# norlab-ulaval/norlab_icp_mapper

Hardware: AMD Instinct MI355X
Metric: ICP iterations/sec, 100k-pt scan vs 1M-pt map (higher is better)
Workload: dtype f32; 1 GPU; single synthetic 100000-pt scan vs 1000000-pt map, point-to-point ICP, KDTreeMatcher knn 1 maxDist 2.0 epsilon 0, TrimmedDist 0.85, fixed 20 iterations per registration; chain=p2p, scene=box+pillars sigma=0.01 seeds 42/43/44 (SURVEY.md 8d), parallelism=scan-sharded x1, map replicated

## Files before the change

include/icpmi.h:

```cpp
#ifndef ICPMI_H
#define ICPMI_H

#include <stdint.h>

#ifdef __cplusplus
extern "C" {
#endif

#define ICPMI_VERSION 4

typedef struct icpmi_ctx* icpmi_handle;

typedef enum {
    ICPMI_OK = 0,
    ICPMI_ERR_INVALID_ARG = 1,
    ICPMI_ERR_HIP = 2,
    ICPMI_ERR_NO_POINT_TO_MINIMIZE = 3,
    ICPMI_ERR_NO_OUTLIER_TO_FILTER = 4,
    ICPMI_ERR_BOUND = 5,
    ICPMI_ERR_NAN = 6,
    ICPMI_ERR_MISSING_NORMALS = 7,
    ICPMI_ERR_UNSUPPORTED = 8
} icpmi_status;

// ... 39 lines not shown
    int32_t minimizer;
    int32_t force_4dof;
    int32_t force_2d;
    int32_t is_2d;
    int32_t max_iterations;
    int32_t use_differential;
    float   min_diff_rot;
    float   min_diff_trans;
    int32_t smooth_length;
    int32_t use_bound;
    float   max_rot_norm;
    float   max_trans_norm;
    float   grid_cell;
    int32_t use_graph;
    int32_t profile;
    int32_t fuse_solve;
    int32_t knn_wg_from;
    int32_t sel_window_off;
    int32_t epsilon_approx;
    int32_t covariance;
    float   sensor_std_dev;
    union {
        int32_t var_dist;
        int32_t reserved[2];
    };
} icpmi_config;

typedef struct {
    int32_t iterations;
    int32_t stop_reason;
    int64_t pairs;
// ... 190 lines not shown
```

norlab_icp_mapper_amd/_capi.py:

```python
import ctypes as C
import os

_HERE = os.path.dirname(os.path.abspath(__file__))
LIB_PATH = os.path.join(_HERE, "libicpmi.so")

ICPMI_OK = 0
ERR_INVALID_ARG, ERR_HIP, ERR_NO_POINT_TO_MINIMIZE, ERR_NO_OUTLIER_TO_FILTER = 1, 2, 3, 4
ERR_BOUND, ERR_NAN, ERR_MISSING_NORMALS, ERR_UNSUPPORTED = 5, 6, 7, 8
MIN_IDENTITY, MIN_POINT_TO_POINT, MIN_POINT_TO_PLANE = 0, 1, 2
OUT_MAXDIST, OUT_MINDIST, OUT_MEDIANDIST, OUT_TRIMMEDDIST, OUT_SURFACENORMAL = 1, 2, 3, 4, 5
OUT_GENERICDESCRIPTOR, OUT_ROBUST, OUT_VARTRIMMEDDIST = 6, 7, 8
GEN_SOURCE_READING, GEN_SOFT, GEN_LARGER = 1, 2, 4
ROBUST_FCT = {"cauchy": 0, "welsch": 1, "sc": 2, "gm": 3, "tukey": 4, "huber": 5, "L1": 6, "student": 7}
ROBUST_SCALE = {"none": 0, "mad": 1, "berg": 2, "std": 3}
ROBUST_DIST = {"point2point": 0, "point2plane": 1}
STOP_NONE, STOP_COUNTER, STOP_DIFFERENTIAL = 0, 1, 2


class Outlier(C.Structure):
    _fields_ = [("type", C.c_int32), ("param", C.c_float), ("iparam", C.c_int32), ("param2", C.c_float), ("param3", C.c_float)]


class _ConfigTail(C.Union):
    _fields_ = [("var_dist", C.c_int32), ("reserved", C.c_int32 * 2)]
# ... 11 lines not shown
        ("minimizer", C.c_int32),
        ("force_4dof", C.c_int32),
        ("force_2d", C.c_int32),
        ("is_2d", C.c_int32),
        ("max_iterations", C.c_int32),
        ("use_differential", C.c_int32),
        ("min_diff_rot", C.c_float),
        ("min_diff_trans", C.c_float),
        ("smooth_length", C.c_int32),
        ("use_bound", C.c_int32),
        ("max_rot_norm", C.c_float),
        ("max_trans_norm", C.c_float),
        ("grid_cell", C.c_float),
        ("use_graph", C.c_int32),
        ("profile", C.c_int32),
        ("fuse_solve", C.c_int32),
        ("knn_wg_from", C.c_int32),
        ("sel_window_off", C.c_int32),
        ("epsilon_approx", C.c_int32),
        ("covariance", C.c_int32),
        ("sensor_std_dev", C.c_float),
        ("tail", _ConfigTail),
    ]


class Stats(C.Structure):
    _fields_ = [
        ("iterations", C.c_int32),
        ("stop_reason", C.c_int32),
        ("pairs", C.c_int64),
        ("point_used_ratio", C.c_float),
# ... 134 lines not shown
```

norlab_icp_mapper_amd/csrc/api.hip:

```cpp
#include "common.h"
#include <cstring>
#include <new>
#include <dlfcn.h>
#include <mutex>
#include <cstdio>

static std::string g_create_error;

namespace {
struct Roctx {
    int (*push)(const char*) = nullptr;
    int (*pop)() = nullptr;
    Roctx()
    {
        const char* e = getenv("ICPMI_ROCTX");
        if (!e || !atoi(e)) return;
        for (const char* name : {"librocprofiler-sdk-roctx.so.1", "librocprofiler-sdk-roctx.so", "/opt/rocm/lib/librocprofiler-sdk-roctx.so.1",
                                 "libroctx64.so.4", "libroctx64.so", "/opt/rocm/lib/libroctx64.so.4"}) {
            void* lib = dlopen(name, RTLD_NOW | RTLD_GLOBAL);
            if (!lib) continue;
            push = (int (*)(const char*))dlsym(lib, "roctxRangePushA");
            pop = (int (*)())dlsym(lib, "roctxRangePop");
            if (push && pop) return;
            push = nullptr; pop = nullptr;
// ... 41 lines not shown
    cfg->n_outlier = 0;
    cfg->minimizer = ICPMI_MIN_POINT_TO_PLANE;
    cfg->max_iterations = 40;
    cfg->use_differential = 0;
    cfg->min_diff_rot = 0.001f;
    cfg->min_diff_trans = 0.001f;
    cfg->smooth_length = 3;
    cfg->use_bound = 0;
    cfg->max_rot_norm = 1.f;
    cfg->max_trans_norm = 1.f;
    cfg->grid_cell = 0.f;
    cfg->use_graph = 1;
    cfg->profile = 0;
    cfg->covariance = 0;
    cfg->sensor_std_dev = 0.01f;
}

static icpmi_status validate_config(const icpmi_config* cfg, std::string& err)
{
    if (cfg->knn < 1 || cfg->knn > ICPMI_MAX_K) { err = "InvalidParameter: knn must be in [1, 32]"; return ICPMI_ERR_INVALID_ARG; }
    if (cfg->var_dist != 0 && cfg->var_dist != 1) { err = "InvalidParameter: var_dist must be 0 or 1"; return ICPMI_ERR_INVALID_ARG; }
    if (!cfg->var_dist && !(cfg->max_dist > 0.f)) { err = "InvalidParameter: maxDist must be > 0"; return ICPMI_ERR_INVALID_ARG; }
    if (cfg->epsilon < 0.f) { err = "InvalidParameter: epsilon must be >= 0"; return ICPMI_ERR_INVALID_ARG; }
    if (cfg->n_outlier < 0 || cfg->n_outlier > ICPMI_MAX_OUTLIER) { err = "InvalidParameter: at most 8 outlier filters"; return ICPMI_ERR_INVALID_ARG; }
    for (int f = 0; f < cfg->n_outlier; ++f) {
        const int t = cfg->outlier[f].type;
        const float p = cfg->outlier[f].param;
        if (t < ICPMI_OUT_MAXDIST || t > ICPMI_OUT_VARTRIMMEDDIST) { err = "InvalidParameter: unknown outlier filter type"; return ICPMI_ERR_INVALID_ARG; }
        if (t == ICPMI_OUT_VARTRIMMEDDIST) {
            const float lo = cfg->outlier[f].param, hi = cfg->outlier[f].param2, lam = cfg->outlier[f].param3;
// ... 177 lines not shown

icpmi_status icpmi_debug_counters(icpmi_handle h, uint64_t out[24])
{
    if (!h || !out) return ICPMI_ERR_INVALID_ARG;
    for (int i = 0; i < 24; ++i) out[i] = h->h_state->dbg[i];
#ifndef ICPMI_NN_TIMING
    out[14] = (uint64_t)h->merge_fast_epochs;
    out[15] = (uint64_t)h->merge_slow_epochs;
    out[16] = (uint64_t)h->oct_respeculated;
    out[17] = (uint64_t)h->raw_view_count;
    out[18] = (uint64_t)(uint32_t)h->ins_count | ((uint64_t)(uint32_t)(h->temp_raw ? h->temp_raw->ins_count : 0) << 32);
    out[19] = (uint64_t)(uint32_t)h->full_count | ((uint64_t)(uint32_t)(h->temp_raw ? h->temp_raw->full_count : 0) << 32);
    out[20] = (uint64_t)h->normals_incremental;
    out[21] = (uint64_t)h->normals_full;
    out[22] = (uint64_t)h->normals_last_searched;
#endif
    return ICPMI_OK;
}

icpmi_status icpmi_debug_last_matches(icpmi_handle h, int64_t n, int32_t k, int32_t* ids, float* d2, float T_used[16])
{
    CHECK_H(h);
    if (n < 1 || k < 1 || !ids || !d2 || !T_used) { h->last_error = "debug_last_matches: bad arguments"; return ICPMI_ERR_INVALID_ARG; }
    if (h->last_match_n == 0) {
        h->last_error = "debug_last_matches: no single registration's matches on this handle (none ran, it failed, or a batch / another call came after it)";
        return ICPMI_ERR_UNSUPPORTED;
    }
    if (n != h->last_match_n || k != h->last_match_k) { h->last_error = "debug_last_matches: n / k differ from the last registration's"; return ICPMI_ERR_INVALID_ARG; }
    const size_t cnt = (size_t)n * k;
    DevBuf<int> d_ids;
// ... 934 lines not shown
```

norlab_icp_mapper_amd/csrc/common.h:

```cpp
#pragma once

#include <hip/hip_runtime.h>
#include <stdint.h>
#include <math.h>
#include <cstring>
#include <string>
#include <vector>
#include <unordered_map>
#include <mutex>
#include <map>
#include <cstdlib>
#include <shared_mutex>

#include "../../include/icpmi.h"

#define ICPMI_NV 32
#define ICPMI_MAX_OUTLIER 8
#define ICPMI_MAX_SMOOTH 16
#define ICPMI_SEL_BINS 2048
#ifndef ICPMI_S2_COPIES
#define ICPMI_S2_COPIES 8
#endif
#define ICPMI_S2_C0 4096
#define ICPMI_S2_F0 (ICPMI_S2_C0 + ICPMI_S2_COPIES * 256)
// ... 354 lines not shown
    bool own_stream = false;
    std::string last_error;
    std::recursive_mutex mu;

    int64_t m = 0;
    float mean[3] = {0, 0, 0};
    GridParams grid{};
    int64_t n_occupied = 0;
    DevArr<float4> d_map_sorted;
    DevArr<float4> d_normals_sorted;
    DevArr<float4> d_map_pn;
    DevArr<unsigned> d_cell_start;
    bool has_normals = false;
    GridLevels levels{};
    DevArr<uint4> d_lvl_tab;
    DevArr<float4> d_lvl_pts[ICPMI_MAXLEV];
    DevArr<unsigned> d_lvl_cs[ICPMI_MAXLEV];
    DevArr<unsigned> d_lvl_pos0[ICPMI_MAXLEV];
    DevArr<unsigned> d_inv;
    DevArr<unsigned> d_lvl_key[ICPMI_MAXLEV];
    DevArr<float4> d_alt_pts[ICPMI_MAXLEV];
    DevArr<unsigned> d_alt_cs[ICPMI_MAXLEV];
    DevArr<unsigned> d_alt_pos0[ICPMI_MAXLEV];
    DevArr<unsigned> d_alt_key[ICPMI_MAXLEV];
    DevArr<float4> d_raw0;
    DevArr<float4> d_alt_raw0;
    DevArr<unsigned> d_ins_dstart0;
    DevArr<float4> d_alt_nsorted;
    DevArr<float4> d_alt_pn;
    DevArr<unsigned> d_ins_key;
    DevArr<unsigned> d_ins_rank;
    bool ins_ready = false;
    bool ins_normals_changed = false;
    double sum_raw[3] = {0, 0, 0};
    float lo_raw[3] = {0, 0, 0}, hi_raw[3] = {0, 0, 0};
    float cell0 = 0.f;
    uint64_t raw_epoch = 0;
    uint64_t temp_raw_epoch = 0; int64_t temp_raw_m = 0;
    uint64_t raw_view_version = 0;
// ... 529 lines not shown
```

norlab_icp_mapper_amd/csrc/map_build.hip:

```cpp
#include "common.h"
#include <cstring>

namespace {

constexpr int RB = 256;

__global__ __launch_bounds__(RB) void stats_kernel(const float4* __restrict__ pts, int64_t m, double* __restrict__ part)
{
    double sx = 0, sy = 0, sz = 0;
    float lo[3] = {INFINITY, INFINITY, INFINITY}, hi[3] = {-INFINITY, -INFINITY, -INFINITY};
    for (int64_t i = (int64_t)blockIdx.x * RB + threadIdx.x; i < m; i += (int64_t)gridDim.x * RB) {
        const float4 p = pts[i];
        sx += p.x; sy += p.y; sz += p.z;
        lo[0] = fminf(lo[0], p.x); lo[1] = fminf(lo[1], p.y); lo[2] = fminf(lo[2], p.z);
        hi[0] = fmaxf(hi[0], p.x); hi[1] = fmaxf(hi[1], p.y); hi[2] = fmaxf(hi[2], p.z);
    }
    __shared__ double sh[RB * 3];
    __shared__ float shlo[RB * 3], shhi[RB * 3];
    const int t = threadIdx.x;
    sh[t] = sx; sh[RB + t] = sy; sh[2 * RB + t] = sz;
    for (int r = 0; r < 3; ++r) { shlo[r * RB + t] = lo[r]; shhi[r * RB + t] = hi[r]; }
    __syncthreads();
    for (int s = RB / 2; s > 0; s >>= 1) {
        if (t < s) {
// ... 731 lines not shown


static GridParams make_grid(const float lo[3], const float hi[3], float cell, float maxabs)
{
    GridParams g;
    g.ox = lo[0]; g.oy = lo[1]; g.oz = lo[2];
    g.cell = cell; g.inv_cell = 1.0f / cell;
    g.slack = cell * 1e-3f + maxabs * 2e-6f;
    g.nx = (int)floorf((hi[0] - lo[0]) * g.inv_cell) + 1;
    g.ny = (int)floorf((hi[1] - lo[1]) * g.inv_cell) + 1;
    g.nz = (int)floorf((hi[2] - lo[2]) * g.inv_cell) + 1;
    g.ncells = g.nx * g.ny * g.nz;
    return g;
}

icpmi_status upload_level_table(icpmi_ctx* c)
{
    GridLevels& L = c->levels;
    uint32_t tab[ICPMI_MAXLEV * 16] = {0};
    auto fbits = [](float f) { uint32_t u; memcpy(&u, &f, 4); return u; };
    for (int l = 0; l < L.nlev; ++l) {
        uint32_t* t = tab + 16 * l;
        const GridParams& gl = L.g[l];
        t[0] = fbits(gl.ox); t[1] = fbits(gl.oy); t[2] = fbits(gl.oz); t[3] = fbits(gl.cell);
        t[4] = fbits(gl.inv_cell); t[5] = fbits(gl.slack); t[6] = (uint32_t)gl.nx; t[7] = (uint32_t)gl.ny;
        t[8] = (uint32_t)gl.nz; t[9] = (uint32_t)gl.ncells;
        const uint64_t pp = (uint64_t)(uintptr_t)L.pts[l], pc = (uint64_t)(uintptr_t)L.cs[l], p0 = (uint64_t)(uintptr_t)L.pos0[l];
        t[10] = (uint32_t)pp; t[11] = (uint32_t)(pp >> 32);
        t[12] = (uint32_t)pc; t[13] = (uint32_t)(pc >> 32); t[14] = (uint32_t)p0; t[15] = (uint32_t)(p0 >> 32);
    }
    if (!c->d_lvl_tab) HIP_TRY(c, c->d_lvl_tab.alloc(ICPMI_MAXLEV * 4));
    return upload_small(c, c->d_lvl_tab, tab, sizeof tab);
}

static icpmi_status map_insert(icpmi_ctx* c, const float4* d_pts, int64_t m0, int64_t m1, const float* d_normals3, bool normals_changed, bool* done)
{
    *done = false;
    static int on = -1, min_m = -1;
    if (on < 0) { on = 1; const char* e = getenv("ICPMI_INSERT_MIN"); min_m = e ? atoi(e) : 0; }
    const int64_t n = m1 - m0;
    GridLevels& L = c->levels;
    if (!on || !c->ins_ready || m0 != c->m || m0 <= 0 || n <= 0 || n > m0 / 2 || m1 < min_m || (d_normals3 != nullptr) != c->has_normals || c->cfg.grid_cell > 0.f) return ICPMI_OK;
    if (c->keep_raw && (d_pts != c->d_raw || (d_normals3 && d_normals3 != c->d_raw_n3))) return ICPMI_OK;
    const int rblocks = (int)std::min<int64_t>((n + RB - 1) / RB, 256);
    if (c->d_red.ensure(c, (size_t)rblocks * 9) != ICPMI_OK) return ICPMI_ERR_HIP;
    hipLaunchKernelGGL(stats_kernel, dim3(rblocks), dim3(RB), 0, c->stream, d_pts + m0, n, c->d_red);
    HIP_TRY(c, hipGetLastError());
// ... 1 lines not shown
    if (read_back(c, part.data(), c->d_red, part.size() * sizeof(double)) != ICPMI_OK) return ICPMI_ERR_HIP;
    double sum[3] = {c->sum_raw[0], c->sum_raw[1], c->sum_raw[2]};
    for (int b = 0; b < rblocks; ++b)
        for (int r = 0; r < 3; ++r) {
            sum[r] += part[(size_t)b * 9 + r];
            const float lo = (float)part[(size_t)b * 9 + 3 + r], hi = (float)part[(size_t)b * 9 + 6 + r];
            const float over = 2.0f * c->levels.g[0].cell;
            if (!(lo >= c->lo_raw[r] - over) || !(hi <= c->hi_raw[r] + over)) return ICPMI_OK;
        }
    float mean[3], clo[3], chi[3], maxabs = 0.f;
    for (int r = 0; r < 3; ++r) {
        mean[r] = c->no_centre ? 0.f : (float)(sum[r] / (double)m1);
        clo[r] = c->lo_raw[r] - mean[r]; chi[r] = c->hi_raw[r] - mean[r];
        maxabs = fmaxf(maxabs, fmaxf(fabsf(clo[r]), fabsf(chi[r])));
    }
    GridParams gnew[ICPMI_MAXLEV];
    for (int l = 0; l < L.nlev; ++l) {
        gnew[l] = make_grid(clo, chi, L.g[l].cell, maxabs);
        if (gnew[l].nx != L.g[l].nx || gnew[l].ny != L.g[l].ny || gnew[l].nz != L.g[l].nz) return ICPMI_OK;
    }
    const bool with_n = d_normals3 != nullptr;
    const bool with_pn = with_n && c->d_map_pn != nullptr && !c->single_level && c->keep_raw;
    if (c->d_ins_key.ensure(c, (size_t)n + 1) != ICPMI_OK || c->d_ins_rank.ensure(c, (size_t)n + 1) != ICPMI_OK) return ICPMI_ERR_HIP;
    const bool twin = !c->no_centre;
    if (twin && !c->d_raw0) return ICPMI_OK;
    if (c->d_inv.ensure(c, (size_t)n + 1) != ICPMI_OK) return ICPMI_ERR_HIP;
    if (c->d_fill.ensure(c, (size_t)L.g[0].ncells + 2) != ICPMI_OK) return ICPMI_ERR_HIP;
    c->fill_clean = false;
    if (c->d_ins_dstart0.ensure(c, (size_t)L.g[0].ncells + 2) != ICPMI_OK) return ICPMI_ERR_HIP;
    if (twin && c->d_alt_raw0.ensure(c, (size_t)m1 + 16) != ICPMI_OK) return ICPMI_ERR_HIP;
    for (int l = 0; l < L.nlev; ++l) {
        if (c->d_alt_pts[l].ensure(c, (size_t)m1 + 16) != ICPMI_OK) return ICPMI_ERR_HIP;
        if (c->d_alt_key[l].ensure(c, (size_t)m1 + 1) != ICPMI_OK) return ICPMI_ERR_HIP;
        if (c->d_alt_cs[l].ensure(c, (size_t)L.g[l].ncells + 2) != ICPMI_OK) return ICPMI_ERR_HIP;
        if (l > 0 && c->d_alt_pos0[l].ensure(c, (size_t)m1 + 1) != ICPMI_OK) return ICPMI_ERR_HIP;
    }
    if (with_n && c->d_alt_nsorted.ensure(c, (size_t)m1 + 1) != ICPMI_OK) return ICPMI_ERR_HIP;
    if (with_pn && c->d_alt_pn.ensure(c, 2 * (size_t)m1 + 2) != ICPMI_OK) return ICPMI_ERR_HIP;
    const int gb0 = (int)((m0 + 255) / 256), gbn = (int)((n + 255) / 256);
    for (int l = 0; l < L.nlev; ++l) {
        const GridParams& g = gnew[l];
        float4* pts_old = l == 0 ? c->d_map_sorted : c->d_lvl_pts[l];
        unsigned* cs_old = l == 0 ? c->d_cell_start : c->d_lvl_cs[l];
        unsigned* key_old = c->d_lvl_key[l];
        unsigned* dstart = l == 0 ? c->d_ins_dstart0 : c->d_fill;
        HIP_TRY(c, hipMemsetAsync(dstart, 0, ((size_t)g.ncells + 2) * sizeof(unsigned), c->stream));
        hipLaunchKernelGGL(ins_key_kernel, dim3(gbn), dim3(256), 0, c->stream, d_pts, m0, n, mean[0], mean[1], mean[2], g, c->d_ins_key, c->d_ins_rank, dstart);
        if (device_exclusive_scan(c, dstart, g.ncells, (unsigned)n) != ICPMI_OK) return ICPMI_ERR_HIP;
        if (l == 0)
            hipLaunchKernelGGL(ins_move0_kernel, dim3(gb0), dim3(256), 0, c->stream, (const float4*)pts_old, twin ? (const float4*)c->d_raw0 : (const float4*)nullptr,
                               (const unsigned*)key_old, m0, (const unsigned*)dstart, mean[0], mean[1], mean[2], c->d_alt_pts[0],
                               twin ? c->d_alt_raw0 : (float4*)nullptr, c->d_alt_key[0], normals_changed ? d_normals3 : (const float*)nullptr,
                               (const float4*)c->d_normals_sorted, with_n ? c->d_alt_nsorted : (float4*)nullptr, with_pn ? c->d_alt_pn : (float4*)nullptr);
        else
            hipLaunchKernelGGL(ins_movel_kernel, dim3(gb0), dim3(256), 0, c->stream, (const unsigned*)key_old, (const unsigned*)c->d_lvl_pos0[l], m0,
// ... 5 lines not shown
                           (l == 0 && with_pn) ? c->d_alt_pn : (float4*)nullptr, (l == 0 && twin) ? c->d_alt_raw0 : (float4*)nullptr);
        hipLaunchKernelGGL(ins_cs_kernel, dim3((g.ncells + 1 + 255) / 256), dim3(256), 0, c->stream, (const unsigned*)cs_old, (const unsigned*)dstart, g.ncells + 1, c->d_alt_cs[l],
                           l == 0 ? dstart + g.ncells + 1 : (unsigned*)nullptr);
        HIP_TRY(c, hipGetLastError());
        if (l == 0 && c->h_nocc) HIP_TRY(c, hipMemcpyAsync(c->h_nocc + 1, dstart + g.ncells + 1, sizeof(unsigned), hipMemcpyDeviceToHost, c->stream));
    }
    GridLevels Lnew = L;
    for (int l = 0; l < L.nlev; ++l) {
        Lnew.g[l] = gnew[l];
        Lnew.pts[l] = c->d_alt_pts[l];
        Lnew.cs[l] = c->d_alt_cs[l];
        Lnew.pos0[l] = l == 0 ? nullptr : c->d_alt_pos0[l];
    }
    {
        const GridLevels Lold = L;
        L = Lnew;
        const icpmi_status us = upload_level_table(c);
        const hipError_t se = us == ICPMI_OK ? hipStreamSynchronize(c->stream) : hipSuccess;
        if (us != ICPMI_OK || se != hipSuccess) {
            L = Lold; c->ins_ready = false; c->m = 0; c->m_raw = 0; drop_loop_graphs(c);
            if (us != ICPMI_OK) return us;
            HIP_TRY(c, se);
        }
    }
    swap(c->d_map_sorted, c->d_alt_pts[0]);
    swap(c->d_cell_start, c->d_alt_cs[0]);
    for (int l = 0; l < L.nlev; ++l) swap(c->d_lvl_key[l], c->d_alt_key[l]);
    for (int l = 1; l < L.nlev; ++l) { swap(c->d_lvl_pts[l], c->d_alt_pts[l]); swap(c->d_lvl_cs[l], c->d_alt_cs[l]); swap(c->d_lvl_pos0[l], c->d_alt_pos0[l]); }
    if (twin) swap(c->d_raw0, c->d_alt_raw0);
    if (with_n) swap(c->d_normals_sorted, c->d_alt_nsorted);
    if (with_pn) swap(c->d_map_pn, c->d_alt_pn);
    for (int l = 0; l < L.nlev; ++l) {
        L.g[l] = gnew[l];
        L.pts[l] = l == 0 ? c->d_map_sorted : c->d_lvl_pts[l];
        L.cs[l] = l == 0 ? c->d_cell_start : c->d_lvl_cs[l];
        L.pos0[l] = l == 0 ? nullptr : c->d_lvl_pos0[l];
    }
    c->grid = gnew[0];
    for (int r = 0; r < 3; ++r) { c->mean[r] = mean[r]; c->sum_raw[r] = sum[r]; }
    if (c->h_nocc) { c->n_occupied += c->h_nocc[1]; *c->h_nocc = (unsigned)c->n_occupied; c->nocc_m = m1; }
    c->m = m1;
    c->m_raw = c->keep_raw ? m1 : 0; c->raw_has_normals = c->keep_raw && with_n;
    c->qsorted_n = -1; c->qsorted_src = nullptr;
// ... 169 lines not shown
        if (reaches || tiny) break;
        GridParams gl = make_grid(clo, chi, prev.cell * 2.0f, maxabs);
        if (c->d_lvl_cs[l].ensure(c, (size_t)gl.ncells + 2) != ICPMI_OK) return ICPMI_ERR_HIP;
        if (c->d_lvl_pts[l].ensure(c, (size_t)m + 16) != ICPMI_OK) return ICPMI_ERR_HIP;
        if (c->d_lvl_pos0[l].ensure(c, (size_t)m) != ICPMI_OK) return ICPMI_ERR_HIP;
        if (counts_begin(c, (size_t)gl.ncells + 2) != ICPMI_OK) return ICPMI_ERR_HIP;
        hipLaunchKernelGGL(lvl_key_kernel, dim3(blocks), dim3(256), 0, c->stream, c->d_map_sorted, m, gl, c->d_keys, c->d_fill);
        if (device_scan_counts_to_cursors(c, c->d_fill, c->d_lvl_cs[l], gl.ncells, (unsigned)m) != ICPMI_OK) return ICPMI_ERR_HIP;
        if (want_ins && c->d_lvl_key[l].ensure(c, (size_t)m + 1) != ICPMI_OK) return ICPMI_ERR_HIP;
        hipLaunchKernelGGL(lvl_scatter_kernel, dim3(blocks), dim3(256), 0, c->stream, c->d_map_sorted, m, c->d_keys, c->d_lvl_cs[l] + 1,
                           c->d_lvl_pts[l], c->d_lvl_pos0[l], want_ins ? c->d_lvl_key[l] : (unsigned*)nullptr);
        HIP_TRY(c, hipGetLastError());
        L.g[l] = gl; L.pts[l] = c->d_lvl_pts[l]; L.cs[l] = c->d_lvl_cs[l]; L.pos0[l] = c->d_lvl_pos0[l];
        L.nlev = l + 1;
    }
    { const icpmi_status us = upload_level_table(c); if (us != ICPMI_OK) return us; }
    c->ins_ready = want_ins;
    HIP_TRY(c, hipStreamSynchronize(c->stream));
    if (c->h_nocc && c->nocc_m == m) c->n_occupied = *c->h_nocc;
    c->m = m;
    c->qsorted_n = -1; c->qsorted_src = nullptr;
    drop_loop_graphs(c);
    return ICPMI_OK;
}
```

norlab_icp_mapper_amd/csrc/nn.hip:

```cpp
#include "common.h"

namespace {

constexpr int NN_BLOCK = 256;

typedef __attribute__((address_space(1))) unsigned gunsigned;
typedef float vf4 __attribute__((ext_vector_type(4)));
typedef __attribute__((address_space(1))) vf4 gfloat4;

struct RowR2 {
    float uni;
    const float* __restrict__ row;
    const int* __restrict__ slot_index;
};
__device__ __forceinline__ float r2_uniform(float r) { return r; }
__device__ __forceinline__ float r2_uniform(const RowR2& r) { return r.uni; }
__device__ __forceinline__ float r2_query(float r, bool, const int*, int) { return r; }
__device__ __forceinline__ float r2_query(const RowR2& r, bool ok, const int* __restrict__ qindex, int qi)
{
    return ok ? r.row[qindex ? qindex[qi] : qi] : 0.f;
}
__device__ __forceinline__ const int* r2_slot_index(float) { return nullptr; }
__device__ __forceinline__ const int* r2_slot_index(const RowR2& r) { return r.slot_index; }

// ... 260 lines not shown
            if (mine == win_key && mine != ~0ull) ++head;
            __syncthreads();
        }
    }
}

__global__ __launch_bounds__(256) void ids_kernel(const float4* __restrict__ map, const int* __restrict__ sidx, int64_t count,
                                                  int* __restrict__ ids)
{
    const int64_t i = (int64_t)blockIdx.x * 256 + threadIdx.x;
    if (i >= count) return;
    const int s = sidx[i];
    ids[i] = s < 0 ? -1 : (int)__float_as_uint(map[s].w);
}

#ifdef ICPMI_NN_TIMING
#define NN_TICK(i) do { __builtin_amdgcn_s_waitcnt(0); const long long t_ = clock64(); tacc[i] += t_ - tlast; tlast = t_; } while (0)
#else
#define NN_TICK(i) do { } while (0)
#endif
__device__ __forceinline__ unsigned wave_incl_scan(unsigned v)
{
    v += (unsigned)__builtin_amdgcn_update_dpp(0, (int)v, 0x111, 0xf, 0xf, false);
    v += (unsigned)__builtin_amdgcn_update_dpp(0, (int)v, 0x112, 0xf, 0xf, false);
    v += (unsigned)__builtin_amdgcn_update_dpp(0, (int)v, 0x114, 0xf, 0xf, false);
    v += (unsigned)__builtin_amdgcn_update_dpp(0, (int)v, 0x118, 0xf, 0xf, false);
    v += (unsigned)__builtin_amdgcn_update_dpp(0, (int)v, 0x142, 0xa, 0xf, false);
    v += (unsigned)__builtin_amdgcn_update_dpp(0, (int)v, 0x143, 0xc, 0xf, false);
    return v;
}

#ifndef ICPMI_NN1_WAVES
#define ICPMI_NN1_WAVES 7
#endif
// ... 20 lines not shown
    constexpr int PLB = ICPMI_NN1_PLB;
    const int n = ba.n[blockIdx.y];
    {
        const size_t qo = (size_t)blockIdx.y * (size_t)ba.qstride;
        queries += qo; out_sidx += qo; out_d2 += qo;
        if (qindex) qindex += qo;
        if (match_pt) match_pt += qo;
        if (hist0) hist0 += (size_t)blockIdx.y * ICPMI_SELHIST_WORDS;
        if (Tptr) Tptr = reinterpret_cast<const float*>(reinterpret_cast<const char*>(Tptr) + (size_t)blockIdx.y * sizeof(IcpState));
        st += blockIdx.y;
    }
#ifdef ICPMI_NN_TIMING
    long long tacc[8] = {0, 0, 0, 0, 0, 0, 0, 0};
    long long tlast = clock64();
    const long long t_c0 = tlast, t_w0 = wall_clock64();
#endif
    __shared__ uint4 ltab[ICPMI_MAXLEV * 4];
    __shared__ unsigned lh[256];
    __shared__ uint2 pieces[CAP];
    __shared__ float2 qdec[Q];
    __shared__ float4 qrec[Q];
    __shared__ float2 qaux[Q];
    __shared__ unsigned long long qkey[Q];
    __shared__ unsigned qwin[Q];
    __shared__ float4 qpt[Q];
    __shared__ unsigned s_any, s_total[2];
    const int tid = threadIdx.x;
    const int lane = tid & 63;
    const int wave = tid >> 6;
    const bool w0 = wave == 0;
// ... 32 lines not shown
    if (tid < ICPMI_MAXLEV * 4) ltab[tid] = ltab_mine;
    if (hist0) {
        for (int t = tid; t < 256; t += NT) lh[t] = 0;
        for (int gt = blockIdx.x * NT + tid; gt < 256 + 65536; gt += wgs * NT) hist0[ICPMI_S2_C1 + gt] = 0;
    }
    const bool allow_self = SELF;

    Cand best; best.key = ~0ull; best.sidx = -1;
    bool decided = !active;
    int lev0 = unseeded_lev;
    if (w0) {
        int sp = -1;
        float4 qs = make_float4(0.f, 0.f, 0.f, 0.f);
        if (active && allow_self && st_iter > 0) {
            sp = match_pt ? sp_kept : out_sidx[orig];
            if (sp >= 0) qs = match_pt ? qs_kept : L.pts[0][sp];
        }
        bool want = sp >= 0;
        const float ub2 = sqdist3(p.x, p.y, p.z, qs.x, qs.y, qs.z);
        const float ub = sqrt_up(ub2);
        auto try_level = [&](int lev, const GridParams& gl) {
            const float fx = (p.x - gl.ox) * gl.inv_cell, fy = (p.y - gl.oy) * gl.inv_cell, fz = (p.z - gl.oz) * gl.inv_cell;
            float mfl = fminf(fx - floorf(fx), 1.0f - (fx - floorf(fx)));
            mfl = fminf(mfl, fminf(fy - floorf(fy), 1.0f - (fy - floorf(fy))));
            mfl = fminf(mfl, fminf(fz - floorf(fz), 1.0f - (fz - floorf(fz))));
            if (!(mfl >= 0.f)) mfl = 0.f;
            const float margin = (1.0f + mfl) * gl.cell - 2.0f * gl.slack;
            if (want && ub * inv1e * 1.000001f <= margin) {
                lev0 = lev;
                best.key = pack_key(ub2, __float_as_uint(qs.w));
                best.sidx = sp;
                qpt[slot] = qs;
                want = false;
            }
        };
        try_level(0, L.g[0]);
        for (int lev = 1; lev < L.nlev; ++lev) {
            if (__ballot(want) == 0ull) break;
            try_level(lev, L.g[lev]);
        }
    }
    bool widepre = false;
    if (seed_pre && lev0 > 0 && best.key != ~0ull) { widepre = true; lev0 = 0; }

    int lev = lev0;
    bool did_pre = false;
    if (w0) { qrec[slot] = make_float4(p.x, p.y, p.z, __int_as_float(lev0)); qkey[slot] = best.key; qwin[slot] = (unsigned)best.sidx; }
    NN_TICK(0);
    __syncthreads();
    for (;;) {
        bool run = false, prescan = false;
        if (w0) {
            run = !decided && lev < L.nlev;
            const bool any = __ballot(run) != 0ull;
            if (lane == 0) { s_any = any ? 1u : 0u; s_total[0] = 0u; s_total[1] = 0u; }
            if (any) {
                const int lv = run ? lev : 0;
                const unsigned long long bk = qkey[slot];
                prescan = run && !did_pre && (bk == ~0ull || (widepre && lev == 0));
                float rub2 = INFINITY;
                if (!prescan && bk != ~0ull) {
                    const float slack = __uint_as_float(ltab[4 * lv + 1].y);
                    const float rub = sqrt_up(__uint_as_float((unsigned)(bk >> 32))) * inv1e * 1.000001f + slack;
                    rub2 = rub * rub;
                }
                reinterpret_cast<float*>(&qrec[slot])[3] = __int_as_float(lv);
                qaux[slot] = make_float2(rub2, __int_as_float((run ? 1 : 0) | (prescan ? 2 : 0)));
            }
        }
        __syncthreads();
        if (!s_any) break;
        NN_TICK(1);
        {
            float mf, g_cell, g_slack;
// ... 96 lines not shown
        tacc[6] += 1; tacc[7] += total;
#endif
        for (unsigned i0 = 0; i0 < total; i0 += (unsigned)NT) {
            const unsigned i = i0 + (unsigned)tid;
            const bool has = i < total;
            const uint2 e = pieces[has ? i : 0u];
            const unsigned qsl = e.y & 255u, cnt = has ? e.y >> 8 : 0u;
            const float4 qr = qrec[qsl];
            const uint4 lt2 = ltab[4 * __float_as_int(qr.w) + 2];
            const gfloat4* mp = reinterpret_cast<const gfloat4*>((((unsigned long long)lt2.w << 32) | lt2.z) + (unsigned long long)e.x * 16ull);
            unsigned long long kb = ~0ull;
            unsigned pb = 0;
            float bx = 0.f, by = 0.f, bz = 0.f;
            for (unsigned c0 = 0; c0 < cnt; c0 += 8u) {
                vf4 q[8];
#pragma unroll
                for (int u = 0; u < 8; ++u) q[u] = mp[c0 + u];
#pragma unroll
                for (int u = 0; u < 8; ++u) {
                    const float d2 = sqdist3(qr.x, qr.y, qr.z, q[u].x, q[u].y, q[u].z);
                    const unsigned long long key = pack_key(d2, __float_as_uint(q[u].w));
                    bool ok = c0 + (unsigned)u < cnt;
                    if (!allow_self) ok = ok && d2 > 1.1920929e-07f;
                    if (ok && key < kb) { kb = key; pb = c0 + (unsigned)u; bx = q[u].x; by = q[u].y; bz = q[u].z; }
                }
            }
            if (kb != ~0ull) atomicMin(&qkey[qsl], kb);
            __syncthreads();
            if (kb != ~0ull && __atomic_load_n(&qkey[qsl], __ATOMIC_RELAXED) == kb) {
                qwin[qsl] = (e.x + pb) | (__float_as_uint(qr.w) << 28);
                qpt[qsl] = make_float4(bx, by, bz, __uint_as_float((unsigned)(kb & 0xffffffffull)));
            }
        }
        __syncthreads();
        NN_TICK(3);
        if (w0 && run) {
            const unsigned long long k2 = qkey[slot];
            if (prescan) did_pre = true;
// ... 13 lines not shown
    float bd2 = __uint_as_float((unsigned)(best.key >> 32));
    const bool found = best.key != ~0ull && bd2 <= r2_query(maxr, active, qindex, qi);
    if (!found) bd2 = INFINITY;
    const bool writer = active;
    if (hist0) {
        if (writer && decided && bd2 != INFINITY && bd2 > 0.f) atomicAdd(&lh[__float_as_uint(bd2) >> 24], 1u);
        __syncthreads();
        for (int t = tid; t < 256; t += NT)
            if (lh[t]) atomicAdd(&hist0[ICPMI_S2_C0 + (blockIdx.x % ICPMI_S2_COPIES) * 256 + t], lh[t]);
    }
    if (writer) {
        int bs = -1;
        float4 mpt = make_float4(0.f, 0.f, 0.f, 0.f);
        if (found) {
            const unsigned lvb = (unsigned)best.sidx >> 28, pos = (unsigned)best.sidx & 0x0fffffffu;
            if (lvb == 0) bs = (int)pos;
            else {
                const uint4 d = ltab[4 * lvb + 3];
                bs = (int)reinterpret_cast<const unsigned*>(((unsigned long long)d.w << 32) | d.z)[pos];
            }
            mpt = qpt[slot];
        }
        st_stream(out_sidx + orig, bs);
        st_stream(out_d2 + orig, bd2);
        if (match_pt) st_stream(match_pt + orig, make_float4(mpt.x, mpt.y, mpt.z, __uint_as_float((unsigned)(best.key & 0xffffffffull))));
        if (hist0 && decided && bd2 != INFINITY && bd2 > 0.f) {
            const unsigned bits = __float_as_uint(bd2);
            atomicAdd(&hist0[ICPMI_S2_F0 + (blockIdx.x % ICPMI_S2_FCOPIES) * 65536 + ICPMI_S2_FIDX(bits >> 16)], 1u);
        }
        if (!decided) {
            const unsigned hslot = atomicAdd(&st->hard_count, 1u);
            hard[hslot] = (unsigned)(match_pt ? qi : (qindex ? qindex[qi] : qi));
        }
    }
#ifdef ICPMI_NN_TIMING
    NN_TICK(5);
    if (threadIdx.x == 0 && st_iter > 1 && (blockIdx.x % 7) == 0) {
        atomicMax(&st->dbg[20], (unsigned long long)(clock64() - t_c0));
        atomicMax(&st->dbg[21], (unsigned long long)tacc[7]);
    }
    if (threadIdx.x == 0 && (blockIdx.x % 61) == 0) {
        const int tb = st_iter > 1 ? 8 : 0;
        for (int i = 0; i < 6; ++i) atomicAdd(&st->dbg[tb + i], (unsigned long long)tacc[i]);
        atomicAdd(&st->dbg[tb + 6], (unsigned long long)tacc[6]);
        atomicAdd(&st->dbg[tb + 7], 1ull);
        atomicAdd(&st->dbg[16 + (st_iter > 1 ? 1 : 0)], (unsigned long long)tacc[7]);
        atomicAdd(&st->dbg[22], (unsigned long long)(clock64() - t_c0));
        atomicAdd(&st->dbg[23], (unsigned long long)(wall_clock64() - t_w0));
    }
#endif
// ... 711 lines not shown
    });
    hipLaunchKernelGGL(hard_reset_kernel, dim3(1), dim3(64), 0, c->stream, d_state);
}

icpmi_status nn_launch_k1(icpmi_ctx* c, const float4* d_reading, int64_t n, const float* d_T, const LoopCfg& lc, int allow_self,
                          int* d_sidx, float* d_d2, IcpState* d_state)
{
    c->nn_out_sorted = false;
    {
        const bool sorted = c->batch_cur > 1 || (c->qsorted_n == n && c->qsorted_src == d_reading);
        const float4* q = sorted ? c->d_qsorted : d_reading;
        const int* qi = sorted ? c->d_qindex : nullptr;
        if (n == 0) return ICPMI_OK;
        const GridParams& topg = c->levels.g[c->levels.nlev - 1];
        const bool needs_hard = !std::isfinite(lc.max_dist) || (topg.cell - topg.slack) <= lc.max_dist;
        const int unseeded_lev = 0;
        const bool hard_sorted = needs_hard && allow_self && sorted && c->batch_cur <= 1;
        unsigned* h0 = (needs_hard && !hard_sorted) ? nullptr : c->nn_hist0;
        c->nn_builds_hist0 = h0 != nullptr;
        float4* mp = ((needs_hard && !hard_sorted) || !sorted) ? nullptr : c->nn_match_pt;
        c->nn_out_sorted = mp != nullptr;
        const BatchArgs ba = c->batch_cur > 1 ? c->batch_args : batch_of_one(n);
        const bool seeded = c->nn_iter_hint > 0 && allow_self;
        const int seed_pre = (seeded && c->nn_iter_hint > 1) ? 0 : 1;
#define LAUNCH_WG(S_)                                                                                                           \
    hipLaunchKernelGGL((nn1_wg_kernel<4, S_, decltype(maxr)>), dim3((int)(((n + 63) / 64 + 7) / 8 * 8), ba.nscan), dim3(256), 0, c->stream,    \
                       q, qi, ba, d_T, c->levels, maxr, d_sidx, d_d2, d_state, c->d_hard, h0, mp, c->d_lvl_tab, unseeded_lev, seed_pre, lc.inv1e, lc.err2)
        with_accept_radius(c, lc, nullptr, [&](auto maxr) { if (allow_self) LAUNCH_WG(true); else LAUNCH_WG(false); });
#undef LAUNCH_WG
        const GridParams& top = c->levels.g[c->levels.nlev - 1];
        if (!std::isfinite(lc.max_dist) || (top.cell - top.slack) <= lc.max_dist) {
            if (hard_sorted && mp)
                with_accept_radius(c, lc, qi, [&](auto maxr) {
                    hipLaunchKernelGGL(nn1_hard_kernel<decltype(maxr)>, dim3(512), dim3(NN_BLOCK), 0, c->stream, q, d_T, c->d_map_sorted, (int)c->m,
                                       maxr, allow_self, d_sidx, d_d2, d_state, c->d_hard, mp, c->nn_builds_hist0 ? c->nn_hist0 : (unsigned*)nullptr);
                });
            else
                with_accept_radius(c, lc, nullptr, [&](auto maxr) {
                    hipLaunchKernelGGL(nn1_hard_kernel<decltype(maxr)>, dim3(512), dim3(NN_BLOCK), 0, c->stream, d_reading, d_T, c->d_map_sorted, (int)c->m,
                                       maxr, allow_self, d_sidx, d_d2, d_state, c->d_hard, (float4*)nullptr, (unsigned*)nullptr);
                });
            if (!(hard_sorted && mp)) hipLaunchKernelGGL(hard_reset_kernel, dim3(1), dim3(64), 0, c->stream, d_state);
// ... 90 lines not shown
```

Measured before the change: 23880 iterations/s.

## Add finer half-cell grid level for NN search and predicate tail loads

Builds an extra map grid level at half the base cell size and prepends it to the level hierarchy used by the workgroup NN kernel when epsilon is exact. Unseeded queries start at level 1 so that fine cells bound the candidate scan more tightly. The fine level is also maintained during map insertion. Separately, the 8-point candidate load is rewritten in inline assembly that uses exec masking to skip out-of-range loads. The cost is extra map-build work and memory, plus more complex level indexing. The config field fuse_solve is renamed to fine_level.

Measured after the change: 21500 iterations/s. -10.0%, worse.

```diff
diff --git a/include/icpmi.h b/include/icpmi.h
--- a/include/icpmi.h
+++ b/include/icpmi.h
@@ -77,7 +77,7 @@
     float   grid_cell;
     int32_t use_graph;
     int32_t profile;
-    int32_t fuse_solve;
+    int32_t fine_level;
     int32_t knn_wg_from;
     int32_t sel_window_off;
     int32_t epsilon_approx;
diff --git a/norlab_icp_mapper_amd/_capi.py b/norlab_icp_mapper_amd/_capi.py
--- a/norlab_icp_mapper_amd/_capi.py
+++ b/norlab_icp_mapper_amd/_capi.py
@@ -49,7 +49,7 @@
         ("grid_cell", C.c_float),
         ("use_graph", C.c_int32),
         ("profile", C.c_int32),
-        ("fuse_solve", C.c_int32),
+        ("fine_level", C.c_int32),
         ("knn_wg_from", C.c_int32),
         ("sel_window_off", C.c_int32),
         ("epsilon_approx", C.c_int32),
diff --git a/norlab_icp_mapper_amd/csrc/api.hip b/norlab_icp_mapper_amd/csrc/api.hip
--- a/norlab_icp_mapper_amd/csrc/api.hip
+++ b/norlab_icp_mapper_amd/csrc/api.hip
@@ -79,6 +79,7 @@
     cfg->profile = 0;
     cfg->covariance = 0;
     cfg->sensor_std_dev = 0.01f;
+    cfg->fine_level = 1;
 }
 
 static icpmi_status validate_config(const icpmi_config* cfg, std::string& err)
@@ -286,6 +287,7 @@
     out[20] = (uint64_t)h->normals_incremental;
     out[21] = (uint64_t)h->normals_full;
     out[22] = (uint64_t)h->normals_last_searched;
+    out[23] = h->fine_on ? (uint64_t)h->fine_g.ncells : 0;
 #endif
     return ICPMI_OK;
 }
diff --git a/norlab_icp_mapper_amd/csrc/common.h b/norlab_icp_mapper_amd/csrc/common.h
--- a/norlab_icp_mapper_amd/csrc/common.h
+++ b/norlab_icp_mapper_amd/csrc/common.h
@@ -392,15 +392,20 @@
     bool has_normals = false;
     GridLevels levels{};
     DevArr<uint4> d_lvl_tab;
-    DevArr<float4> d_lvl_pts[ICPMI_MAXLEV];
-    DevArr<unsigned> d_lvl_cs[ICPMI_MAXLEV];
-    DevArr<unsigned> d_lvl_pos0[ICPMI_MAXLEV];
+#define ICPMI_FINE_SLOT ICPMI_MAXLEV
+    bool fine_on = false;
+    GridParams fine_g{};
+    GridLevels levels_fine{};
+    DevArr<uint4> d_lvl_tab_fine;
+    DevArr<float4> d_lvl_pts[ICPMI_MAXLEV + 1];
+    DevArr<unsigned> d_lvl_cs[ICPMI_MAXLEV + 1];
+    DevArr<unsigned> d_lvl_pos0[ICPMI_MAXLEV + 1];
     DevArr<unsigned> d_inv;
-    DevArr<unsigned> d_lvl_key[ICPMI_MAXLEV];
-    DevArr<float4> d_alt_pts[ICPMI_MAXLEV];
-    DevArr<unsigned> d_alt_cs[ICPMI_MAXLEV];
-    DevArr<unsigned> d_alt_pos0[ICPMI_MAXLEV];
-    DevArr<unsigned> d_alt_key[ICPMI_MAXLEV];
+    DevArr<unsigned> d_lvl_key[ICPMI_MAXLEV + 1];
+    DevArr<float4> d_alt_pts[ICPMI_MAXLEV + 1];
+    DevArr<unsigned> d_alt_cs[ICPMI_MAXLEV + 1];
+    DevArr<unsigned> d_alt_pos0[ICPMI_MAXLEV + 1];
+    DevArr<unsigned> d_alt_key[ICPMI_MAXLEV + 1];
     DevArr<float4> d_raw0;
     DevArr<float4> d_alt_raw0;
     DevArr<unsigned> d_ins_dstart0;
diff --git a/norlab_icp_mapper_amd/csrc/map_build.hip b/norlab_icp_mapper_amd/csrc/map_build.hip
--- a/norlab_icp_mapper_amd/csrc/map_build.hip
+++ b/norlab_icp_mapper_amd/csrc/map_build.hip
@@ -769,9 +769,8 @@
     return g;
 }
 
-icpmi_status upload_level_table(icpmi_ctx* c)
-{
-    GridLevels& L = c->levels;
+static icpmi_status upload_one_level_table(icpmi_ctx* c, const GridLevels& L, DevArr<uint4>& d_tab)
+{
     uint32_t tab[ICPMI_MAXLEV * 16] = {0};
     auto fbits = [](float f) { uint32_t u; memcpy(&u, &f, 4); return u; };
     for (int l = 0; l < L.nlev; ++l) {
@@ -784,8 +783,25 @@
         t[10] = (uint32_t)pp; t[11] = (uint32_t)(pp >> 32);
         t[12] = (uint32_t)pc; t[13] = (uint32_t)(pc >> 32); t[14] = (uint32_t)p0; t[15] = (uint32_t)(p0 >> 32);
     }
-    if (!c->d_lvl_tab) HIP_TRY(c, c->d_lvl_tab.alloc(ICPMI_MAXLEV * 4));
-    return upload_small(c, c->d_lvl_tab, tab, sizeof tab);
+    if (!d_tab) HIP_TRY(c, d_tab.alloc(ICPMI_MAXLEV * 4));
+    return upload_small(c, d_tab, tab, sizeof tab);
+}
+
+static icpmi_status upload_level_tables(icpmi_ctx* c, const float4* fine_pts, const unsigned* fine_cs, const unsigned* fine_pos0)
+{
+    const icpmi_status us = upload_one_level_table(c, c->levels, c->d_lvl_tab);
+    if (us != ICPMI_OK || !c->fine_on) return us;
+    GridLevels& F = c->levels_fine;
+    const GridLevels& L = c->levels;
+    F.nlev = L.nlev + 1;
+    F.g[0] = c->fine_g; F.pts[0] = fine_pts; F.cs[0] = fine_cs; F.pos0[0] = fine_pos0;
+    for (int l = 0; l < L.nlev; ++l) { F.g[l + 1] = L.g[l]; F.pts[l + 1] = L.pts[l]; F.cs[l + 1] = L.cs[l]; F.pos0[l + 1] = L.pos0[l]; }
+    return upload_one_level_table(c, F, c->d_lvl_tab_fine);
+}
+
+icpmi_status upload_level_table(icpmi_ctx* c)
+{
+    return upload_level_tables(c, c->d_lvl_pts[ICPMI_FINE_SLOT], c->d_lvl_cs[ICPMI_FINE_SLOT], c->d_lvl_pos0[ICPMI_FINE_SLOT]);
 }
 
 static icpmi_status map_insert(icpmi_ctx* c, const float4* d_pts, int64_t m0, int64_t m1, const float* d_normals3, bool normals_changed, bool* done)
@@ -817,10 +833,20 @@
         clo[r] = c->lo_raw[r] - mean[r]; chi[r] = c->hi_raw[r] - mean[r];
         maxabs = fmaxf(maxabs, fmaxf(fabsf(clo[r]), fabsf(chi[r])));
     }
-    GridParams gnew[ICPMI_MAXLEV];
-    for (int l = 0; l < L.nlev; ++l) {
-        gnew[l] = make_grid(clo, chi, L.g[l].cell, maxabs);
-        if (gnew[l].nx != L.g[l].nx || gnew[l].ny != L.g[l].ny || gnew[l].nz != L.g[l].nz) return ICPMI_OK;
+    constexpr int FS = ICPMI_FINE_SLOT;
+    int slots[ICPMI_MAXLEV + 1], nslots = 0;
+    for (int l = 0; l < L.nlev; ++l) slots[nslots++] = l;
+#ifndef ICPMI_FINE_INSERT
+#define ICPMI_FINE_INSERT 1
+#endif
+    const bool merge_fine = c->fine_on && ICPMI_FINE_INSERT;
+    if (merge_fine) slots[nslots++] = FS;
+    GridParams gnew[ICPMI_MAXLEV + 1];
+    for (int i = 0; i < nslots; ++i) {
+        const int l = slots[i];
+        const GridParams& gold = l == FS ? c->fine_g : L.g[l];
+        gnew[l] = make_grid(clo, chi, gold.cell, maxabs);
+        if (gnew[l].nx != gold.nx || gnew[l].ny != gold.ny || gnew[l].nz != gold.nz) return ICPMI_OK;
     }
     const bool with_n = d_normals3 != nullptr;
     const bool with_pn = with_n && c->d_map_pn != nullptr && !c->single_level && c->keep_raw;
@@ -828,20 +854,22 @@
     const bool twin = !c->no_centre;
     if (twin && !c->d_raw0) return ICPMI_OK;
     if (c->d_inv.ensure(c, (size_t)n + 1) != ICPMI_OK) return ICPMI_ERR_HIP;
-    if (c->d_fill.ensure(c, (size_t)L.g[0].ncells + 2) != ICPMI_OK) return ICPMI_ERR_HIP;
+    if (c->d_fill.ensure(c, (size_t)(merge_fine ? c->fine_g.ncells : L.g[0].ncells) + 2) != ICPMI_OK) return ICPMI_ERR_HIP;
     c->fill_clean = false;
     if (c->d_ins_dstart0.ensure(c, (size_t)L.g[0].ncells + 2) != ICPMI_OK) return ICPMI_ERR_HIP;
     if (twin && c->d_alt_raw0.ensure(c, (size_t)m1 + 16) != ICPMI_OK) return ICPMI_ERR_HIP;
-    for (int l = 0; l < L.nlev; ++l) {
+    for (int i = 0; i < nslots; ++i) {
+        const int l = slots[i];
         if (c->d_alt_pts[l].ensure(c, (size_t)m1 + 16) != ICPMI_OK) return ICPMI_ERR_HIP;
         if (c->d_alt_key[l].ensure(c, (size_t)m1 + 1) != ICPMI_OK) return ICPMI_ERR_HIP;
-        if (c->d_alt_cs[l].ensure(c, (size_t)L.g[l].ncells + 2) != ICPMI_OK) return ICPMI_ERR_HIP;
+        if (c->d_alt_cs[l].ensure(c, (size_t)gnew[l].ncells + 2) != ICPMI_OK) return ICPMI_ERR_HIP;
         if (l > 0 && c->d_alt_pos0[l].ensure(c, (size_t)m1 + 1) != ICPMI_OK) return ICPMI_ERR_HIP;
     }
     if (with_n && c->d_alt_nsorted.ensure(c, (size_t)m1 + 1) != ICPMI_OK) return ICPMI_ERR_HIP;
     if (with_pn && c->d_alt_pn.ensure(c, 2 * (size_t)m1 + 2) != ICPMI_OK) return ICPMI_ERR_HIP;
     const int gb0 = (int)((m0 + 255) / 256), gbn = (int)((n + 255) / 256);
-    for (int l = 0; l < L.nlev; ++l) {
+    for (int i = 0; i < nslots; ++i) {
+        const int l = slots[i];
         const GridParams& g = gnew[l];
         float4* pts_old = l == 0 ? c->d_map_sorted : c->d_lvl_pts[l];
         unsigned* cs_old = l == 0 ? c->d_cell_start : c->d_lvl_cs[l];
@@ -877,19 +905,22 @@
     }
     {
         const GridLevels Lold = L;
+        const GridParams fine_old = c->fine_g;
         L = Lnew;
-        const icpmi_status us = upload_level_table(c);
+        c->fine_on = merge_fine;
+        if (merge_fine) c->fine_g = gnew[FS];
+        const icpmi_status us = upload_level_tables(c, c->d_alt_pts[FS], c->d_alt_cs[FS], c->d_alt_pos0[FS]);
         const hipError_t se = us == ICPMI_OK ? hipStreamSynchronize(c->stream) : hipSuccess;
         if (us != ICPMI_OK || se != hipSuccess) {
-            L = Lold; c->ins_ready = false; c->m = 0; c->m_raw = 0; drop_loop_graphs(c);
+            L = Lold; c->fine_g = fine_old; c->ins_ready = false; c->m = 0; c->m_raw = 0; drop_loop_graphs(c);
             if (us != ICPMI_OK) return us;
             HIP_TRY(c, se);
         }
     }
     swap(c->d_map_sorted, c->d_alt_pts[0]);
     swap(c->d_cell_start, c->d_alt_cs[0]);
-    for (int l = 0; l < L.nlev; ++l) swap(c->d_lvl_key[l], c->d_alt_key[l]);
-    for (int l = 1; l < L.nlev; ++l) { swap(c->d_lvl_pts[l], c->d_alt_pts[l]); swap(c->d_lvl_cs[l], c->d_alt_cs[l]); swap(c->d_lvl_pos0[l], c->d_alt_pos0[l]); }
+    for (int i = 0; i < nslots; ++i) swap(c->d_lvl_key[slots[i]], c->d_alt_key[slots[i]]);
+    for (int i = 1; i < nslots; ++i) { const int l = slots[i]; swap(c->d_lvl_pts[l], c->d_alt_pts[l]); swap(c->d_lvl_cs[l], c->d_alt_cs[l]); swap(c->d_lvl_pos0[l], c->d_alt_pos0[l]); }
     if (twin) swap(c->d_raw0, c->d_alt_raw0);
     if (with_n) swap(c->d_normals_sorted, c->d_alt_nsorted);
     if (with_pn) swap(c->d_map_pn, c->d_alt_pn);
@@ -1089,6 +1120,25 @@
         L.g[l] = gl; L.pts[l] = c->d_lvl_pts[l]; L.cs[l] = c->d_lvl_cs[l]; L.pos0[l] = c->d_lvl_pos0[l];
         L.nlev = l + 1;
     }
+    c->fine_on = false;
+    if (c->cfg.fine_level && c->keep_raw && !c->single_level && !c->is_raw_index && !(c->cfg.grid_cell > 0.f) && L.nlev < ICPMI_MAXLEV) {
+        constexpr int FS = ICPMI_FINE_SLOT;
+        const GridParams gf = make_grid(clo, chi, g.cell * 0.5f, maxabs);
+        if ((double)gf.nx * (double)gf.ny * (double)gf.nz <= MAX_CELLS) {
+            if (c->d_lvl_cs[FS].ensure(c, (size_t)gf.ncells + 2) != ICPMI_OK) return ICPMI_ERR_HIP;
+            if (c->d_lvl_pts[FS].ensure(c, (size_t)m + 16) != ICPMI_OK) return ICPMI_ERR_HIP;
+            if (c->d_lvl_pos0[FS].ensure(c, (size_t)m) != ICPMI_OK) return ICPMI_ERR_HIP;
+            if (counts_begin(c, (size_t)gf.ncells + 2) != ICPMI_OK) return ICPMI_ERR_HIP;
+            hipLaunchKernelGGL(lvl_key_kernel, dim3(blocks), dim3(256), 0, c->stream, c->d_map_sorted, m, gf, c->d_keys, c->d_fill);
+            if (device_scan_counts_to_cursors(c, c->d_fill, c->d_lvl_cs[FS], gf.ncells, (unsigned)m) != ICPMI_OK) return ICPMI_ERR_HIP;
+            if (want_ins && c->d_lvl_key[FS].ensure(c, (size_t)m + 1) != ICPMI_OK) return ICPMI_ERR_HIP;
+            hipLaunchKernelGGL(lvl_scatter_kernel, dim3(blocks), dim3(256), 0, c->stream, c->d_map_sorted, m, c->d_keys, c->d_lvl_cs[FS] + 1,
+                               c->d_lvl_pts[FS], c->d_lvl_pos0[FS], want_ins ? c->d_lvl_key[FS] : (unsigned*)nullptr);
+            HIP_TRY(c, hipGetLastError());
+            c->fine_g = gf;
+            c->fine_on = true;
+        }
+    }
     { const icpmi_status us = upload_level_table(c); if (us != ICPMI_OK) return us; }
     c->ins_ready = want_ins;
     HIP_TRY(c, hipStreamSynchronize(c->stream));
diff --git a/norlab_icp_mapper_amd/csrc/nn.hip b/norlab_icp_mapper_amd/csrc/nn.hip
--- a/norlab_icp_mapper_amd/csrc/nn.hip
+++ b/norlab_icp_mapper_amd/csrc/nn.hip
@@ -298,10 +298,21 @@
     ids[i] = s < 0 ? -1 : (int)__float_as_uint(map[s].w);
 }
 
-#ifdef ICPMI_NN_TIMING
+#if defined(ICPMI_NN_TIMING) && (ICPMI_NN_TIMING + 0) == 2
+#define ICPMI_NN_COUNTERS 1
+#endif
+#if defined(ICPMI_NN_TIMING) && !defined(ICPMI_NN_COUNTERS)
 #define NN_TICK(i) do { __builtin_amdgcn_s_waitcnt(0); const long long t_ = clock64(); tacc[i] += t_ - tlast; tlast = t_; } while (0)
 #else
 #define NN_TICK(i) do { } while (0)
+#endif
+#ifdef ICPMI_NN_COUNTERS
+#define NN_COUNT(ok_, ld_) do { n_ok += (ok_); n_ld += (ld_); } while (0)
+#else
+#define NN_COUNT(ok_, ld_) do { } while (0)
+#endif
+#ifndef ICPMI_NN1_PRED
+#define ICPMI_NN1_PRED 1
 #endif
 __device__ __forceinline__ unsigned wave_incl_scan(unsigned v)
 {
@@ -352,6 +363,12 @@
     long long tacc[8] = {0, 0, 0, 0, 0, 0, 0, 0};
     long long tlast = clock64();
     const long long t_c0 = tlast, t_w0 = wall_clock64();
+    (void)t_c0; (void)t_w0;
+#endif
+#ifdef ICPMI_NN_COUNTERS
+    unsigned n_ok = 0, n_ld = 0;
+    __shared__ unsigned s_cnt[8];
+    if (threadIdx.x < 8) s_cnt[threadIdx.x] = 0u;
 #endif
     __shared__ uint4 ltab[ICPMI_MAXLEV * 4];
     __shared__ unsigned lh[256];
@@ -414,7 +431,7 @@
         float4 qs = make_float4(0.f, 0.f, 0.f, 0.f);
         if (active && allow_self && st_iter > 0) {
             sp = match_pt ? sp_kept : out_sidx[orig];
-            if (sp >= 0) qs = match_pt ? qs_kept : L.pts[0][sp];
+            if (sp >= 0) qs = match_pt ? qs_kept : (unseeded_lev ? L.pts[1] : L.pts[0])[sp];
         }
         bool want = sp >= 0;
         const float ub2 = sqdist3(p.x, p.y, p.z, qs.x, qs.y, qs.z);
@@ -429,7 +446,7 @@
             if (want && ub * inv1e * 1.000001f <= margin) {
                 lev0 = lev;
                 best.key = pack_key(ub2, __float_as_uint(qs.w));
-                best.sidx = sp;
+                best.sidx = (int)((unsigned)sp | ((unsigned)unseeded_lev << 28));
                 qpt[slot] = qs;
                 want = false;
             }
@@ -441,7 +458,7 @@
         }
     }
     bool widepre = false;
-    if (seed_pre && lev0 > 0 && best.key != ~0ull) { widepre = true; lev0 = 0; }
+    if (seed_pre && lev0 > unseeded_lev && best.key != ~0ull) { widepre = true; lev0 = unseeded_lev; }
 
     int lev = lev0;
     bool did_pre = false;
@@ -457,7 +474,7 @@
             if (any) {
                 const int lv = run ? lev : 0;
                 const unsigned long long bk = qkey[slot];
-                prescan = run && !did_pre && (bk == ~0ull || (widepre && lev == 0));
+                prescan = run && !did_pre && (bk == ~0ull || (widepre && lev == unseeded_lev));
                 float rub2 = INFINITY;
                 if (!prescan && bk != ~0ull) {
                     const float slack = __uint_as_float(ltab[4 * lv + 1].y);
@@ -584,14 +601,65 @@
             float bx = 0.f, by = 0.f, bz = 0.f;
             for (unsigned c0 = 0; c0 < cnt; c0 += 8u) {
                 vf4 q[8];
+#if ICPMI_NN1_PRED == 1
+                {
+                    const gfloat4* a = mp + c0;
+                    const unsigned c0u = (unsigned)__builtin_amdgcn_readfirstlane((int)c0);
+                    unsigned long long ex;
+                    unsigned t;
+                    asm volatile("s_mov_b64 %[ex], exec\n\t"
+                                 "global_load_dwordx4 %[q0], %[a], off\n\t"
+                                 "s_add_u32 %[t], %[c0], 1\n\t"
+                                 "v_cmpx_lt_u32_e64 vcc, %[t], %[cnt]\n\t"
+                                 "global_load_dwordx4 %[q1], %[a], off offset:16\n\t"
+                                 "s_add_u32 %[t], %[c0], 2\n\t"
+                                 "v_cmpx_lt_u32_e64 vcc, %[t], %[cnt]\n\t"
+                                 "global_load_dwordx4 %[q2], %[a], off offset:32\n\t"
+                                 "s_add_u32 %[t], %[c0], 3\n\t"
+                                 "v_cmpx_lt_u32_e64 vcc, %[t], %[cnt]\n\t"
+                                 "global_load_dwordx4 %[q3], %[a], off offset:48\n\t"
+                                 "s_add_u32 %[t], %[c0], 4\n\t"
+                                 "v_cmpx_lt_u32_e64 vcc, %[t], %[cnt]\n\t"
+                                 "global_load_dwordx4 %[q4], %[a], off offset:64\n\t"
+                                 "s_add_u32 %[t], %[c0], 5\n\t"
+                                 "v_cmpx_lt_u32_e64 vcc, %[t], %[cnt]\n\t"
+                                 "global_load_dwordx4 %[q5], %[a], off offset:80\n\t"
+                                 "s_add_u32 %[t], %[c0], 6\n\t"
+                                 "v_cmpx_lt_u32_e64 vcc, %[t], %[cnt]\n\t"
+                                 "global_load_dwordx4 %[q6], %[a], off offset:96\n\t"
+                                 "s_add_u32 %[t], %[c0], 7\n\t"
+                                 "v_cmpx_lt_u32_e64 vcc, %[t], %[cnt]\n\t"
+                                 "global_load_dwordx4 %[q7], %[a], off offset:112\n\t"
+                                 "s_mov_b64 exec, %[ex]\n\t"
+                                 "s_waitcnt vmcnt(0)"
+                                 : [q0] "=&v"(q[0]), [q1] "=&v"(q[1]), [q2] "=&v"(q[2]), [q3] "=&v"(q[3]), [q4] "=&v"(q[4]), [q5] "=&v"(q[5]),
+                                   [q6] "=&v"(q[6]), [q7] "=&v"(q[7]), [ex] "=&s"(ex), [t] "=&s"(t)
+                                 : [a] "v"(a), [cnt] "v"(cnt), [c0] "s"(c0u)
+                                 : "vcc", "scc");
+                }
+#elif ICPMI_NN1_PRED == 2
+#pragma unroll
+                for (int u = 0; u < 4; ++u) q[u] = mp[c0 + u];
+                const bool more = __ballot(cnt > c0 + 4u) != 0ull;
+#pragma unroll
+                for (int u = 4; u < 8; ++u) q[u] = more ? mp[c0 + u] : q[0];
+#else
 #pragma unroll
                 for (int u = 0; u < 8; ++u) q[u] = mp[c0 + u];
+#endif
 #pragma unroll
                 for (int u = 0; u < 8; ++u) {
                     const float d2 = sqdist3(qr.x, qr.y, qr.z, q[u].x, q[u].y, q[u].z);
                     const unsigned long long key = pack_key(d2, __float_as_uint(q[u].w));
                     bool ok = c0 + (unsigned)u < cnt;
                     if (!allow_self) ok = ok && d2 > 1.1920929e-07f;
+#if ICPMI_NN1_PRED == 1
+                    NN_COUNT(ok ? 1u : 0u, c0 + (unsigned)u < cnt ? 1u : 0u);
+#elif ICPMI_NN1_PRED == 2
+                    NN_COUNT(ok ? 1u : 0u, (u >= 4 && !more) ? 0u : 1u);
+#else
+                    NN_COUNT(ok ? 1u : 0u, 1u);
+#endif
                     if (ok && key < kb) { kb = key; pb = c0 + (unsigned)u; bx = q[u].x; by = q[u].y; bz = q[u].z; }
                 }
             }
@@ -635,11 +703,9 @@
         float4 mpt = make_float4(0.f, 0.f, 0.f, 0.f);
         if (found) {
             const unsigned lvb = (unsigned)best.sidx >> 28, pos = (unsigned)best.sidx & 0x0fffffffu;
-            if (lvb == 0) bs = (int)pos;
-            else {
-                const uint4 d = ltab[4 * lvb + 3];
-                bs = (int)reinterpret_cast<const unsigned*>(((unsigned long long)d.w << 32) | d.z)[pos];
-            }
+            const uint4 d = ltab[4 * lvb + 3];
+            if ((d.z | d.w) == 0u) bs = (int)pos;
+            else bs = (int)reinterpret_cast<const unsigned*>(((unsigned long long)d.w << 32) | d.z)[pos];
             mpt = qpt[slot];
         }
         st_stream(out_sidx + orig, bs);
@@ -654,7 +720,18 @@
             hard[hslot] = (unsigned)(match_pt ? qi : (qindex ? qindex[qi] : qi));
         }
     }
-#ifdef ICPMI_NN_TIMING
+#ifdef ICPMI_NN_COUNTERS
+    if ((blockIdx.x % 61) == 0) {
+        if (n_ok) atomicAdd(&s_cnt[0], n_ok);
+        if (n_ld) atomicAdd(&s_cnt[1], n_ld);
+        if (active) { atomicAdd(&s_cnt[3], 1u); atomicAdd(&s_cnt[4 + (!decided || lev > 3 ? 3 : lev)], 1u); }
+        __syncthreads();
+        if (threadIdx.x < 8) {
+            const unsigned v = threadIdx.x == 2 ? (unsigned)tacc[7] : s_cnt[threadIdx.x];
+            if (v) atomicAdd(&st->dbg[(st_iter > 1 ? 8 : 0) + threadIdx.x], (unsigned long long)v);
+        }
+    }
+#elif defined(ICPMI_NN_TIMING)
     NN_TICK(5);
     if (threadIdx.x == 0 && st_iter > 1 && (blockIdx.x % 7) == 0) {
         atomicMax(&st->dbg[20], (unsigned long long)(clock64() - t_c0));
@@ -1396,7 +1473,10 @@
         if (n == 0) return ICPMI_OK;
         const GridParams& topg = c->levels.g[c->levels.nlev - 1];
         const bool needs_hard = !std::isfinite(lc.max_dist) || (topg.cell - topg.slack) <= lc.max_dist;
-        const int unseeded_lev = 0;
+        const bool fine = c->fine_on && lc.inv1e == 1.0f && lc.err2 == 1.0f;
+        const GridLevels& lv = fine ? c->levels_fine : c->levels;
+        const uint4* lvtab = fine ? c->d_lvl_tab_fine : c->d_lvl_tab;
+        const int unseeded_lev = fine ? 1 : 0;
         const bool hard_sorted = needs_hard && allow_self && sorted && c->batch_cur <= 1;
         unsigned* h0 = (needs_hard && !hard_sorted) ? nullptr : c->nn_hist0;
         c->nn_builds_hist0 = h0 != nullptr;
@@ -1407,7 +1487,7 @@
         const int seed_pre = (seeded && c->nn_iter_hint > 1) ? 0 : 1;
 #define LAUNCH_WG(S_)                                                                                                           \
     hipLaunchKernelGGL((nn1_wg_kernel<4, S_, decltype(maxr)>), dim3((int)(((n + 63) / 64 + 7) / 8 * 8), ba.nscan), dim3(256), 0, c->stream,    \
-                       q, qi, ba, d_T, c->levels, maxr, d_sidx, d_d2, d_state, c->d_hard, h0, mp, c->d_lvl_tab, unseeded_lev, seed_pre, lc.inv1e, lc.err2)
+                       q, qi, ba, d_T, lv, maxr, d_sidx, d_d2, d_state, c->d_hard, h0, mp, lvtab, unseeded_lev, seed_pre, lc.inv1e, lc.err2)
         with_accept_radius(c, lc, nullptr, [&](auto maxr) { if (allow_self) LAUNCH_WG(true); else LAUNCH_WG(false); });
 #undef LAUNCH_WG
         const GridParams& top = c->levels.g[c->levels.nlev - 1];
```
